# wongzbb/DiffMa-Diffusion-Mamba

Hardware: AMD Instinct MI355X
Metric: diffusion-steps/sec (DiffMa-L/2, 224x224, training; samples*steps/s) (higher is better)
Workload: dtype bf16 autocast (fp32 master weights, fp32 scan state); 1 GPU; DiffMa-L/2 DDP training step, 4x28x28 latents (196 tokens), batch 512/GPU; global_batch=512, seq_len=196, parallelism=dp1, gemm_tuning=file, world_size_seen_by_rccl=1

## Files before the change

diffma-diffusion-mamba_amd/csrc/scan_bwd.hip:

```cpp
#include "dm_common.h"
namespace dm {
int scan_bwd_f32(const dm_scan_bwd_args& a, const dm_scan_bwd_args* second, hipStream_t st);
int scan_bwd_bf16(const dm_scan_bwd_args& a, const dm_scan_bwd_args* second, hipStream_t st);
int scan_bwd_f16(const dm_scan_bwd_args& a, const dm_scan_bwd_args* second, hipStream_t st);
bool scan_bwd_takes_two(const dm_scan_bwd_args& a);

static int check_scan_bwd(const dm_scan_bwd_args& a) {
    if (!a.u || !a.delta || !a.dout || !a.A || !a.B || !a.C || !a.du || !a.ddelta || !a.dBC_partial || !a.dA_partial) {
        set_error("dm_selective_scan_bwd: null tensor pointer"); return DM_ERR_ARG;
    }
    if ((a.z != nullptr) != (a.dz != nullptr)) { set_error("dm_selective_scan_bwd: dz must be given iff z is"); return DM_ERR_ARG; }
    if (a.nseq <= 0 || a.dim <= 0 || a.seqlen <= 0 || a.ngroups <= 0) { set_error("dm_selective_scan_bwd: non-positive size"); return DM_ERR_ARG; }
    if (a.nseq > 65535) { set_error("dm_selective_scan_bwd: nseq %d > 65535", a.nseq); return DM_ERR_ARG; }
    if (a.ckpt_every != DM_SCAN_CKPT_EVERY) { set_error("dm_selective_scan_bwd: ckpt_every must be %d", DM_SCAN_CKPT_EVERY); return DM_ERR_ARG; }
    if (!a.ckpt) { set_error("dm_selective_scan_bwd: ckpt (the checkpoints written by dm_selective_scan_fwd) is required"); return DM_ERR_ARG; }
    if (a.ckpt && a.ckpt_dtype != (a.io_dtype == DM_BF16 ? DM_BF16 : DM_F32)) {
        set_error("dm_selective_scan_bwd: ckpt_dtype must be DM_BF16 for bf16 I/O and DM_F32 otherwise"); return DM_ERR_DTYPE;
    }
    if (a.u_sd != 1 || a.dt_sd != 1 || a.do_sd != 1 || a.du_sd != 1 || a.ddt_sd != 1 || (a.z && (a.z_sd != 1 || a.dz_sd != 1)) ||
        a.B_sn != 1 || a.C_sn != 1) {
        set_error("dm_selective_scan_bwd: needs token-major tensors (channel stride 1, state stride 1)"); return DM_ERR_LAYOUT;
    }
    if (a.dim % a.ngroups != 0 || (a.ngroups > 1 && (a.dim / a.ngroups) % WAVE != 0)) {
        set_error("dm_selective_scan_bwd: dim/ngroups must be a multiple of 64"); return DM_ERR_LAYOUT;
    }
    if (a.batch_per_dir > 0 && a.nseq % a.batch_per_dir != 0) { set_error("dm_selective_scan_bwd: nseq %% batch_per_dir != 0"); return DM_ERR_ARG; }
    if ((a.flags & DM_FLAG_DELTA_ACTIVATED) && (a.z || !a.z_row_index || a.dstate != 16 || (a.flags & (DM_FLAG_A_SHARED | DM_FLAG_DELTA_SOFTPLUS)))) {
        set_error("dm_selective_scan_bwd: DM_FLAG_DELTA_ACTIVATED is built for the mixer's call pattern (no z, row indices, d_state 16, no A_SHARED / DELTA_SOFTPLUS)");
        return DM_ERR_ARG;
    }
    if ((a.z_row_index == nullptr) != (a.out_row_index == nullptr)) {
        set_error("dm_selective_scan_bwd: z_row_index and out_row_index must both be set or both be NULL"); return DM_ERR_ARG;
    }
    return DM_OK;
}
static bool pairs_scan_bwd(const dm_scan_bwd_args& x, const dm_scan_bwd_args& y) {
    using A = dm_scan_bwd_args;
    return scan_bwd_takes_two(x) && mix_congruent(x, y, &A::u, &A::delta, &A::z, &A::dout, &A::B, &A::C, &A::A, &A::D, &A::delta_bias,
                                                  &A::z_row_index, &A::out_row_index, &A::ckpt, &A::du, &A::ddelta, &A::dz,
                                                  &A::dBC_partial, &A::dA_partial, &A::dD_partial, &A::dbias_partial);
}
static int run_scan_bwd(const dm_scan_bwd_args& a, const dm_scan_bwd_args* second, hipStream_t st) {
    switch (a.io_dtype) {
        case DM_F32: return scan_bwd_f32(a, second, st);
        case DM_BF16: return scan_bwd_bf16(a, second, st);
        case DM_F16: return scan_bwd_f16(a, second, st);
        default: set_error("dm_selective_scan_bwd: bad io_dtype %d", a.io_dtype); return DM_ERR_DTYPE;
    }
}
}

extern "C" int dm_selective_scan_bwd(const dm_scan_bwd_args* args, void* stream) {
    using namespace dm;
    if (!args) { set_error("dm_selective_scan_bwd: null args"); return DM_ERR_ARG; }
    const int rc = check_scan_bwd(*args);
    return rc ? rc : run_scan_bwd(*args, nullptr, (hipStream_t)stream);
}

extern "C" int dm_selective_scan_bwd_n(const dm_scan_bwd_args* args, int n, void* stream) {
    return dm::mix_run_n("dm_selective_scan_bwd_n", args, n, stream, dm::check_scan_bwd, dm::pairs_scan_bwd, dm::run_scan_bwd);
}
```

diffma-diffusion-mamba_amd/csrc/scan_bwd_impl.h:

```cpp
#pragma once
#include <type_traits>
#include "scan_bwd_step.h"

namespace dm {

constexpr int BWD_CK = 8;
constexpr int BWD_WAVES = 4;

__device__ __forceinline__ void swap32(float& a, float& b) {
    auto r = __builtin_amdgcn_permlane32_swap(__float_as_uint(a), __float_as_uint(b), false, false);
    a = __uint_as_float(r[0]);
    b = __uint_as_float(r[1]);
}
__device__ __forceinline__ void swap16(float& a, float& b) {
    auto r = __builtin_amdgcn_permlane16_swap(__float_as_uint(a), __float_as_uint(b), false, false);
    a = __uint_as_float(r[0]);
    b = __uint_as_float(r[1]);
}
template <int M>
__device__ __forceinline__ void lane_group_reduce(float (&v)[M]) {
    static_assert(M % 4 == 0, "need at least 2 states per lane");
#pragma unroll
    for (int i = 0; i < M / 2; ++i) { swap32(v[2 * i], v[2 * i + 1]); v[i] = v[2 * i] + v[2 * i + 1]; }
#pragma unroll
    for (int i = 0; i < M / 4; ++i) { swap16(v[2 * i], v[2 * i + 1]); v[i] = v[2 * i] + v[2 * i + 1]; }
}

typedef __attribute__((address_space(3))) const float* lds_cfptr;
typedef __attribute__((address_space(3))) const f32x4* lds_cf4ptr;
__device__ __forceinline__ lds_cfptr lds_opaque(lds_cfptr chunk_base) {
    asm volatile("" : "+v"(chunk_base));
    return chunk_base;
}
template <int NS>
__device__ __forceinline__ void lds_ld_vec(float (&v)[NS], lds_cfptr row) {
    if constexpr (NS % 4 == 0) {
#pragma unroll
        for (int k = 0; k < NS / 4; ++k) {
            const f32x4 t = ((lds_cf4ptr)row)[k];
            v[4 * k] = t.x; v[4 * k + 1] = t.y; v[4 * k + 2] = t.z; v[4 * k + 3] = t.w;
        }
    } else {
#pragma unroll
        for (int k = 0; k < NS; ++k) v[k] = row[k];
    }
}

template <typename T, typename TBC, int N, int SPLIT, bool HAS_Z, bool IDX, int DMODE, bool ASH = false>
__global__ __launch_bounds__(64 * BWD_WAVES) __attribute__((amdgpu_waves_per_eu(N <= 16 ? 2 : 1))) void scan_bwd_kernel(const dm_scan_bwd_args p) {
    constexpr int NS = N / SPLIT, NPL = NS / 2, CW = WAVE / SPLIT, CK = BWD_CK, SUB = DM_SCAN_CKPT_EVERY, M = 2 * NS, R = M / 4;
    constexpr int ES = (int)sizeof(T);
    constexpr bool MFMA_RED = std::is_same<T, bf16_t>::value && M % 16 == 0 && SPLIT <= 2;
    constexpr bool HALVES = MFMA_RED && SPLIT == 1 && N == 16;
    constexpr int NH = HALVES ? 2 : 1, NPH = NPL / NH;
    constexpr bool CACHE_A = HALVES && !ASH;
    constexpr bool LDS_AHEAD = HALVES && !HAS_Z;
    static_assert(N % SPLIT == 0 && NS % 2 == 0, "d_state/SPLIT must be even");
    static_assert(CK % SUB == 0, "chunk must be a whole number of sub-chunks");
    static_assert(R % 4 == 0, "lane-group totals are stored 4 registers at a time");
    constexpr int RED_HALF = WAVE * 4 + 4 * 8;
    constexpr int RED_ROW = (R / 4) * RED_HALF;
    __shared__ __attribute__((aligned(16))) float red_lds[BWD_WAVES][CK][RED_ROW];
    __shared__ __attribute__((aligned(16))) float bc_lds[2][CK][2 * N];

    const int tid = threadIdx.x;
    const int wave = tid >> 6, lane = tid & 63;
    const int c = lane / SPLIT, q = lane % SPLIT;
    const int d_raw = (blockIdx.x * BWD_WAVES + wave) * CW + c;
    const bool active = d_raw < p.dim;
    const int d = active ? d_raw : p.dim - 1;
    const int s = blockIdx.y;
    const int L = p.seqlen;
    const int bpd = (p.batch_per_dir > 0) ? p.batch_per_dir : p.nseq;
    const int dir = s / bpd;
    const int sb = s - dir * bpd;
    const int grp = (blockIdx.x * BWD_WAVES * CW) / (p.dim / p.ngroups);
    const int nwg = gridDim.x;
    const int nchunk = (L + CK - 1) / CK;

    const rsrc_t r_u = make_rsrc((const T*)p.u + (int64_t)s * p.u_ss);
    const rsrc_t r_dt = make_rsrc((const T*)p.delta + (int64_t)s * p.dt_ss);
    const rsrc_t r_z = make_rsrc(HAS_Z ? (const T*)p.z + (int64_t)sb * p.z_ss : nullptr);
    const rsrc_t r_g = make_rsrc((const T*)p.dout + (int64_t)((IDX && !(p.flags & DM_FLAG_DOUT_PER_SEQ)) ? sb : s) * p.do_ss);
    const rsrc_t r_du = make_rsrc_2g((T*)p.du + (int64_t)s * p.du_ss);
    const rsrc_t r_ddt = make_rsrc_2g((T*)p.ddelta + (int64_t)s * p.ddt_ss);
    const rsrc_t r_dz = make_rsrc_2g(HAS_Z ? (T*)p.dz + (int64_t)s * p.dz_ss : nullptr);
    const TBC* __restrict__ Bg = (const TBC*)p.B + (int64_t)s * p.B_ss + (int64_t)grp * p.B_sg;
    const TBC* __restrict__ Cg = (const TBC*)p.C + (int64_t)s * p.C_ss + (int64_t)grp * p.C_sg;
    constexpr bool CK_PACKED = std::is_same<T, bf16_t>::value;
    constexpr int CK_ROWS = CK_PACKED ? N / 2 : N;
    const int nck = (L + SUB - 1) / SUB;
    const rsrc_t r_ck = make_rsrc_2g(p.ckpt ? (const uint32_t*)p.ckpt + (int64_t)s * nck * CK_ROWS * p.dim : nullptr);
    const rsrc_t r_dbc = make_rsrc_2g(p.dBC_partial + (int64_t)s * L * gridDim.x * (2 * N));
    const int vo = d * ES;
    const int vo_st = (active && q == 0) ? vo : BIO_OOB;
    const int vo_ck = CK_PACKED ? (d * 4 + q * (CK_ROWS / SPLIT / 4) * p.dim * 4) * 4 : (d + q * (CK_ROWS / SPLIT) * p.dim) * 4;
    const int sl_u = (int)p.u_sl * ES, sl_dt = (int)p.dt_sl * ES, sl_z = (int)p.z_sl * ES, sl_g = (int)p.do_sl * ES;
    const int sl_du = (int)p.du_sl * ES, sl_ddt = (int)p.ddt_sl * ES, sl_dz = (int)p.dz_sl * ES;
    const int i_B_sl = (int)p.B_sl, i_C_sl = (int)p.C_sl;
    const cptr<int32_t> zidx = IDX ? as_const(p.z_row_index + (int64_t)dir * L) : nullptr;
    const cptr<int32_t> oidx = IDX ? as_const(p.out_row_index + (int64_t)dir * L) : nullptr;

    f32x2 A2[NPL];
#pragma unroll
    for (int k = 0; k < NPL; ++k) {
        A2[k].x = p.A[(int64_t)d * N + q * NS + 2 * k] * LOG2E;
        A2[k].y = p.A[(int64_t)d * N + q * NS + 2 * k + 1] * LOG2E;
    }
    const float Dv = p.D ? p.D[d] : 0.0f;
    const float bias = p.delta_bias ? p.delta_bias[d] : 0.0f;

    f32x2 carry[NPL], dA[NPL];
#pragma unroll
    for (int k = 0; k < NPL; ++k) { carry[k] = (f32x2){0.f, 0.f}; dA[k] = (f32x2){0.f, 0.f}; }
    float dD_acc = 0.f, dbias_acc = 0.f;

    u32x4_t sel_lo, sel_hi;
    if (MFMA_RED) mfma_selectors(lane, sel_lo, sel_hi);
    const int red_slot = lane * 4 + (lane >> 4) * 8;

    constexpr int BC_PER_THREAD = (CK * 2 * N + 64 * BWD_WAVES - 1) / (64 * BWD_WAVES);
    auto fetch_bc = [&](int chunk, uint32_t(&v)[BC_PER_THREAD]) {
#pragma unroll
        for (int i = 0; i < BC_PER_THREAD; ++i) {
            int e = tid + i * 64 * BWD_WAVES;
            e = (e < CK * 2 * N) ? e : CK * 2 * N - 1;
            const int j = e / (2 * N), cc = e % (2 * N);
            int l = chunk * CK + j;
            l = (l < L) ? l : L - 1;
            const TBC* src = (cc < N) ? Bg + l * i_B_sl + cc : Cg + l * i_C_sl + (cc - N);
            v[i] = io<TBC>::ld_raw(src);
        }
    };
    auto stash_bc = [&](int b, const uint32_t(&v)[BC_PER_THREAD]) {
#pragma unroll
        for (int i = 0; i < BC_PER_THREAD; ++i) {
            const int e = tid + i * 64 * BWD_WAVES;
            if (e < CK * 2 * N) bc_lds[b][e / (2 * N)][e % (2 * N)] = io<TBC>::cv(v[i]);
        }
    };
    auto flush_dbc = [&](int chunk) {
        const int l0 = chunk * CK;
        if constexpr (HALVES) {
            static_assert(CK * 2 * N == 64 * BWD_WAVES, "one output per thread");
            const int tq = tid & 3, g4 = (tid >> 2) & 7, j = tid >> 5;
            const float* base = &red_lds[0][j][(g4 >> 2) * RED_HALF + (16 * (g4 & 3) + 4 * tq) * 4 + (g4 & 3) * 8];
            f32x4 acc4 = {0.f, 0.f, 0.f, 0.f};
#pragma unroll
            for (int w = 0; w < BWD_WAVES; ++w)
#pragma unroll
                for (int t = 0; t < 4; ++t) acc4 += *reinterpret_cast<const f32x4*>(base + w * (CK * RED_ROW) + t * 4);
#pragma unroll
            for (int i = 0; i < 4; ++i) {
                float v = acc4[i];
                v += dpp<DPP_QUAD_SWAP>(v);
                v += dpp<DPP_QUAD_HALF>(v);
                acc4[i] = v;
            }
            const float mine = tq == 0 ? acc4[0] : (tq == 1 ? acc4[1] : (tq == 2 ? acc4[2] : acc4[3]));
            const int V = 4 * g4 + tq;
            const int col = (V & 8) ? N + 8 * (V >> 4) + (V & 7) : 8 * (V >> 4) + (V & 7);
            const int vo_p = (l0 + j < L) ? (((l0 + j) * nwg + (int)blockIdx.x) * (2 * N) + col) * 4 : BIO_OOB;
            __builtin_amdgcn_raw_buffer_store_b32(__float_as_uint(mine), r_dbc, vo_p, 0, 0);
            return;
        }
#pragma unroll
        for (int it = 0; it < BC_PER_THREAD; ++it) {
            const int e_ = tid + it * 64 * BWD_WAVES;
            const bool in = e_ < CK * 2 * N;
            const int e = in ? e_ : 0;
            const int j = e / (2 * N), cc = e % (2 * N);
            const int vo_p = (in && l0 + j < L) ? (((l0 + j) * nwg + (int)blockIdx.x) * (2 * N) + cc) * 4 : BIO_OOB;
            float acc = 0.f;
            const int n = (cc < N) ? cc : cc - N;
            const int qq = n / NS;
            const int vidx = (cc < N) ? n % NS : NS + n % NS;
            const int lane0 = (MFMA_RED ? 16 * ((vidx & 15) >> 2) : 32 * (vidx & 1) + 16 * ((vidx >> 1) & 1)) + qq;
            const int reg = MFMA_RED ? 4 * (vidx >> 4) + (vidx & 3) : (vidx >> 2);
#pragma unroll
            for (int w = 0; w < BWD_WAVES; ++w)
#pragma unroll
                for (int t = 0; t < 16 / SPLIT; ++t) acc += red_lds[w][j][(reg >> 2) * RED_HALF + (lane0 + SPLIT * t) * 4 + (lane0 >> 4) * 8 + (reg & 3)];
            __builtin_amdgcn_raw_buffer_store_b32(__float_as_uint(acc), r_dbc, vo_p, 0, 0);
        }
    };
    {
        uint32_t v[BC_PER_THREAD];
        fetch_bc(nchunk - 1, v);
        stash_bc(0, v);
    }
    __syncthreads();

    constexpr int H0W = CK_PACKED ? NPL : 2 * NPL;
    auto load_state = [&](int ci, uint32_t(&w)[H0W]) {
        const int slot_ = ckpt_slot(ci, L);
        const int vo_ = (slot_ < 0 || !p.ckpt) ? BIO_OOB : vo_ck;
        const int slot = slot_ < 0 ? 0 : slot_;
        if constexpr (CK_PACKED) {
            bio_ld_words<H0W>(w, r_ck, vo_, slot * p.dim * (N / 2) * 4, p.dim * 16);
        } else {
#pragma unroll
            for (int k = 0; k < NPL; ++k) {
                w[2 * k] = __builtin_amdgcn_raw_buffer_load_b32(r_ck, vo_, ((slot * N + 2 * k) * p.dim) * 4, 0);
                w[2 * k + 1] = __builtin_amdgcn_raw_buffer_load_b32(r_ck, vo_, ((slot * N + 2 * k + 1) * p.dim) * 4, 0);
            }
        }
    };
    auto unpack_state = [&](f32x2(&h)[NPH], const uint32_t(&w)[H0W], int hf) {
        unpack_ckpt<CK_PACKED>(h, w, hf * NPH);
    };
    static_assert(SUB == 4, "row-table entries of a sub-chunk travel in one 4-entry SGPR vector");
    constexpr int NSC = CK / SUB;
    typedef int i32x4_t __attribute__((ext_vector_type(4)));
    auto load_rows = [&](cptr<int32_t> tab, int ci) -> i32x4_t {
        const int lb = ci < 0 ? 0 : ci * SUB;
        i32x4_t r = {0, 0, 0, 0};
#pragma unroll
        for (int i = 0; i < SUB; ++i) {
            const int l = (lb + i < L) ? lb + i : L - 1;
            r[i] = IDX ? tab[(uint32_t)l] : l;
        }
        return r;
    };
    typename bio<T>::raw_t ru[SUB], rd[SUB], rg[SUB], rz[HAS_Z ? SUB : 1];
    uint32_t ck_nx[H0W];
    i32x4_t orow_is = load_rows(oidx, nchunk * NSC - 1), zrow_is = {0, 0, 0, 0};
    if (HAS_Z) zrow_is = load_rows(zidx, nchunk * NSC - 1);
    auto issue_sub = [&](int ci) {
        const int lb = ci < 0 ? 0 : ci * SUB;
#pragma unroll
        for (int i = 0; i < SUB; ++i) {
            const int l = (lb + i < L) ? lb + i : L - 1;
            ru[i] = bio<T>::ld_raw(r_u, vo, l * sl_u);
            rd[i] = bio<T>::ld_raw(r_dt, vo, l * sl_dt);
            if (HAS_Z) rz[i] = bio<T>::ld_raw(r_z, vo, zrow_is[i] * sl_z);
            rg[i] = bio<T>::ld_raw(r_g, vo, orow_is[i] * sl_g);
        }
        load_state(ci, ck_nx);
        orow_is = load_rows(oidx, ci - 1);
        if (HAS_Z) zrow_is = load_rows(zidx, ci - 1);
    };
    uint32_t ck_end[H0W];
    load_state(nchunk * NSC, ck_end);
    f32x2 hend[HALVES ? NH : 1][NPH];
    if constexpr (HALVES) {
#pragma unroll
        for (int hf = 0; hf < NH; ++hf) unpack_state(hend[hf], ck_end, hf);
    }
    i32x4_t zrow_nx = zrow_is;
    issue_sub(nchunk * NSC - 1);

    int buf = 0;
    for (int ch = nchunk - 1; ch >= 0; --ch) {
        const int l0 = ch * CK;
        const lds_cfptr bc_chunk = (lds_cfptr)(&bc_lds[0][0][0]) + (buf * CK * 2 * N + q * NS);
        uint32_t bc_next[BC_PER_THREAD];
        fetch_bc(ch > 0 ? ch - 1 : 0, bc_next);
#pragma unroll
        for (int sc = NSC - 1; sc >= 0; --sc) {
            const int ci = ch * NSC + sc;
            float uu[SUB], dl[SUB], zz[SUB], gg[SUB];
            uint32_t ck_cur[H0W];
            const i32x4_t zrow = zrow_nx;
#pragma unroll
            for (int i = 0; i < SUB; ++i) {
                const bool valid = (l0 + sc * SUB + i) < L;
                uu[i] = bio<T>::cv(ru[i]);
                dl[i] = activate_delta<DMODE>(bio<T>::cv(rd[i]), bias);
                zz[i] = HAS_Z ? bio<T>::cv(rz[i]) : 0.f;
                gg[i] = (valid && active) ? bio<T>::cv(rg[i]) : 0.f;
            }
#pragma unroll
            for (int k = 0; k < H0W; ++k) ck_cur[k] = ck_nx[k];
            zrow_nx = zrow_is;
            issue_sub(ci - 1);
            f32x2 GB2s[SUB], dlA2s[SUB], yp2s[HAS_Z ? SUB : 1];
#pragma unroll
            for (int hf = 0; hf < NH; ++hf) {
            const lds_cfptr bc_rec = lds_opaque(bc_chunk);
            auto fwd_step = [&](f32x2(&h)[NPH], int i, f32x2(&keep)[NPH]) {
                float Bv[2 * NPH];
                const lds_cfptr brow = bc_rec + ((sc * SUB + i) * 2 * N + hf * 2 * NPH);
                lds_ld_vec<2 * NPH>(Bv, brow);
                const float dlo = CACHE_A ? dl[i] : opaque(dl[i]);
                const float du = dlo * uu[i];
                const float a_sh = decay_shared<ASH>(A2[0], dlo);
#pragma unroll
                for (int k = 0; k < NPH; ++k) {
                    const f32x2 a = decay_pair<ASH>(A2[hf * NPH + k], dlo, a_sh);
                    if (CACHE_A) keep[k] = a;
                    recompute_pair(h[k], a, (f32x2){Bv[2 * k], Bv[2 * k + 1]}, du);
                }
            };
            f32x2 h[NPH];
            unpack_state(h, ck_cur, hf);
            f32x2 hs[SUB][NPH];
            f32x2 aa[CACHE_A ? SUB - 1 : 1][NPH];
#pragma unroll
            for (int i = 0; i < SUB; ++i) {
#pragma unroll
                for (int k = 0; k < NPH; ++k) hs[i][k] = h[k];
                if (i < SUB - 1) fwd_step(h, i, aa[CACHE_A ? i : 0]);
            }
            if constexpr (HALVES) {
#pragma unroll
                for (int k = 0; k < NPH; ++k) { h[k] = hend[hf][k]; hend[hf][k] = hs[0][k]; }
            } else {
                unpack_state(h, ck_end, hf);
            }
            const lds_cfptr bc_swp = lds_opaque(bc_chunk);
            float Bn[2 * NPH], Cn[2 * NPH];
            if constexpr (LDS_AHEAD) {
// ... 34 lines not shown
#pragma unroll
                for (int k = 0; k < NPH; ++k) {
                    const int kk = hf * NPH + k;
                    const f32x2 bb = {Bv[2 * k], Bv[2 * k + 1]}, cc = {Cv[2 * k], Cv[2 * k + 1]};
                    const f32x2 a = (CACHE_A && i < SUB - 1) ? aa[CACHE_A ? i : 0][k] : decay_pair<ASH>(A2[kk], dlo, a_rev);
                    f32x2 dBp, dCp;
                    adjoint_pair<HAS_Z, true>(h[k], hs[i][k], carry[kk], dA[kk], yp2, GB2, dlA2, A2[kk], a, bb, cc, gy, du, dlo, dBp, dCp);
                    if constexpr (MFMA_RED) {
                        pk_all[k] = pack_bf16(dBp);
                        pk_all[NPH + k] = pack_bf16(dCp);
                    } else {
                        red[2 * k] = dBp.x;
                        red[2 * k + 1] = dBp.y;
                        red[NS + 2 * k] = dCp.x;
                        red[NS + 2 * k + 1] = dCp.y;
                    }
                }
                if (hf < NH - 1) { GB2s[i] = GB2; dlA2s[i] = dlA2; if (HAS_Z) yp2s[i] = yp2; }
                if (hf == NH - 1) {
                float ddl, duv, ypre, dDi;
                step_outputs<DMODE, SPLIT>(yp2, GB2, dlA2, uu[i], dlo, gy, Dv, ddl, duv, ypre, dDi);
                if (q == 0) {
                    dD_acc += dDi;
                    dbias_acc += ddl;
                }
                const int vo_s = valid ? vo_st : BIO_OOB;
                bio<T>::st_cv(r_du, vo_s, l * sl_du, duv);
                bio<T>::st_cv(r_ddt, vo_s, l * sl_ddt, ddl);
                if (HAS_Z) {
                    const float dzv = gate_grad(g, ypre, zz[i], sz);
                    bio<T>::st_cv(r_dz, vo_s, zrow[i] * sl_dz, dzv);
                }
                }
                if constexpr (MFMA_RED) {
#pragma unroll
                    for (int g16 = 0; g16 < M / 16 / NH; ++g16)
                        *reinterpret_cast<f32x4*>(&red_lds[wave][j][(NH == 2 ? hf : g16) * RED_HALF + red_slot]) = group_sum16(sel_lo, sel_hi, pk_all + 8 * g16);
                } else {
                    lane_group_reduce<M>(red);
#pragma unroll
                    for (int r4 = 0; r4 < R / 4; ++r4)
                        *reinterpret_cast<f32x4*>(&red_lds[wave][j][r4 * RED_HALF + red_slot]) = (f32x4){red[4 * r4], red[4 * r4 + 1], red[4 * r4 + 2], red[4 * r4 + 3]};
                }
            }
            }
#pragma unroll
            for (int k = 0; k < H0W; ++k) ck_end[k] = ck_cur[k];
        }
        __syncthreads();
        flush_dbc(ch);
        if (ch > 0) stash_bc(buf ^ 1, bc_next);
        __syncthreads();
        buf ^= 1;
    }
    if (active) {
        const int64_t pss_a = p.part_ss ? p.part_ss : (int64_t)p.dim * N, pss_d = p.part_ss ? p.part_ss : (int64_t)p.dim;
        float* dAp = p.dA_partial + (int64_t)s * pss_a + (int64_t)d * N + q * NS;
#pragma unroll
        for (int k = 0; k < NPL; ++k) {
            dAp[2 * k] = dA[k].x;
            dAp[2 * k + 1] = dA[k].y;
        }
        if (q == 0) {
            if (p.dD_partial) p.dD_partial[(int64_t)s * pss_d + d] = dD_acc;
            if (p.dbias_partial) p.dbias_partial[(int64_t)s * pss_d + d] = dbias_acc;
        }
    }
}

template <int N> struct bwd_split { static constexpr int value = N >= 32 ? (N >= 64 ? N / 16 : 2) : 1; };

template <int N, bool HAS_Z, bool IDX, typename F>
static void with_bwd_variant(int flags, F f) {
    const bool sp = (flags & DM_FLAG_DELTA_SOFTPLUS) != 0;
    if constexpr ((N == 16 || N == 64 || N == 128) && HAS_Z && IDX) {
        if ((flags & DM_FLAG_A_SHARED) && sp) return f(std::integral_constant<int, 1>{}, std::true_type{});
    }
    if constexpr (N == 16 && !HAS_Z && IDX) {
        if (flags & DM_FLAG_DELTA_ACTIVATED) return f(std::integral_constant<int, 2>{}, std::false_type{});
    }
    if (sp) f(std::integral_constant<int, 1>{}, std::false_type{});
    else f(std::integral_constant<int, 0>{}, std::false_type{});
}

template <typename T, typename TBC, int N>
static int launch_bwd(const dm_scan_bwd_args& a, hipStream_t st) {
    constexpr int SPLIT = bwd_split<N>::value, WGCH = (WAVE / SPLIT) * BWD_WAVES;
    dim3 grid((a.dim + WGCH - 1) / WGCH, a.nseq);
    with_z_idx(a, [&](auto hz, auto ix) {
        with_bwd_variant<N, hz.value, ix.value>(a.flags, [&](auto dmode, auto ash) {
            hipLaunchKernelGGL((scan_bwd_kernel<T, TBC, N, SPLIT, hz.value, ix.value, dmode.value, ash.value>), grid, dim3(WAVE * BWD_WAVES), 0, st, a);
        });
    });
    return launch_status("dm_selective_scan_bwd");
}

template <typename T, typename TBC>
static int bwd_dispatch_n(const dm_scan_bwd_args& a, hipStream_t st) {
    switch (a.dstate) {
        case 16: return launch_bwd<T, TBC, 16>(a, st);
#ifndef DM_FAST_BUILD
        case 8: return launch_bwd<T, TBC, 8>(a, st);
        case 32: return launch_bwd<T, TBC, 32>(a, st);
        case 64: return launch_bwd<T, TBC, 64>(a, st);
        case 128: return launch_bwd<T, TBC, 128>(a, st);
#endif
        default: set_error("dm_selective_scan_bwd: d_state=%d not instantiated (8,16,32,64,128)", a.dstate); return DM_ERR_DSTATE;
    }
}

template <typename T>
static int bwd_dispatch_bc(const dm_scan_bwd_args& a, hipStream_t st) {
    if (a.bc_dtype == DM_F32) return bwd_dispatch_n<T, float>(a, st);
    if (a.bc_dtype == a.io_dtype) return bwd_dispatch_n<T, T>(a, st);
    set_error("dm_selective_scan_bwd: bc_dtype %d must be fp32 or equal io_dtype %d", a.bc_dtype, a.io_dtype);
    return DM_ERR_DTYPE;
}

}
```

diffma-diffusion-mamba_amd/hip_ops.py:

```python
from __future__ import annotations

import ctypes
import os
import threading

import torch

from . import _lib
from ._lib import (DM_BF16, DM_F16, DM_F32, DM_FLAG_A_SHARED, DM_FLAG_DELTA_ACTIVATED, DM_FLAG_DX_MERGED, DM_FLAG_PARTIAL_COMPACT, DM_FLAG_OUT_ACCUMULATE, DM_FLAG_DELTA_SOFTPLUS, DM_FLAG_DOUT_PER_SEQ, DM_FLAG_SCAN_CHUNKED, DM_FLAG_SCAN_SEQUENTIAL, DM_FLAG_SILU, dm_blend_args, dm_gate_head_args, dm_dtproj_bwd_args, dm_conv_bwd_args, dm_rmsnorm_merge_args, dm_colsum_args, dm_sum_partials_args,
                   dm_conv_fwd_args, dm_conv_xproj_bwd_args, dm_conv_xproj_fwd_args, dm_diffusion_step_args, dm_ln_mod_args, dm_ssd_bwd_args, dm_ssd_fwd_args, dm_merge_args, dm_gate_bwd_args, dm_dtproj_args, dm_scan_bwd_args, dm_scan_fwd_args, dm_gemm_args, dm_repack_args, dm_training_loss_args)

_DT = {torch.float32: DM_F32, torch.bfloat16: DM_BF16, torch.float16: DM_F16}
SCAN_CKPT_EVERY = _lib.DM_SCAN_CKPT_EVERY


def union_length(intervals):
    total, cur_s, cur_e = 0.0, None, None
    for s0, e0 in sorted(intervals):
        if cur_e is None or s0 > cur_e:
            if cur_e is not None:
                total += cur_e - cur_s
            cur_s, cur_e = s0, e0
        else:
            cur_e = max(cur_e, e0)
# ... 210 lines not shown
    return a


def scan_fwd(u, delta, A, Bm, Cm, D=None, z=None, delta_bias=None, delta_softplus=True, *,
             z_row_index=None, out_row_index=None, batch_per_dir=0, out=None, ckpt=None,
             ckpt_every=SCAN_CKPT_EVERY, last_state=None, ngroups=1, a_shared=False, variant=None, acc_dirs=False,
             delta_activated=False):
    _require_gpu(u, delta, A, Bm, Cm, z)
    S, L, Dm = u.shape
    N = A.shape[1]
    if acc_dirs:
        Bd = batch_per_dir
        ndir = S // Bd
        if out is None:
            out = torch.empty((Bd, L, Dm), dtype=u.dtype, device=u.device)
        for k in range(ndir):
            sl = slice(k * Bd, (k + 1) * Bd)
            _scan_fwd_launch(u[sl], delta[sl], A, Bm[sl], Cm[sl], D, z, delta_bias, delta_softplus, z_row_index[k:k + 1],
                             out_row_index[k:k + 1], 0, out, None if ckpt is None else ckpt[sl], ckpt_every, None, ngroups, False,
                             "sequential", k > 0)
        return out
    if out is None:
        out = torch.empty((S, L, Dm), dtype=u.dtype, device=u.device)
    return _scan_fwd_launch(u, delta, A, Bm, Cm, D, z, delta_bias, delta_softplus, z_row_index, out_row_index, batch_per_dir, out, ckpt,
                            ckpt_every, last_state, ngroups, a_shared, variant, False, delta_activated)


def _scan_fwd_launch(u, delta, A, Bm, Cm, D, z, delta_bias, delta_softplus, z_row_index, out_row_index, batch_per_dir, out, ckpt,
                     ckpt_every, last_state, ngroups, a_shared, variant, accumulate, delta_activated=False):
    S, L, Dm = u.shape
    N = A.shape[1]
    A, D, delta_bias = _f32c(A), _f32c(D), _f32c(delta_bias)
    a = _scan_args(dm_scan_fwd_args(), u, delta, A, Bm, Cm, D, z, delta_bias, delta_softplus, delta_activated, z_row_index, out_row_index,
                   batch_per_dir, ckpt, ckpt_every, ngroups, a_shared, variant, DM_FLAG_OUT_ACCUMULATE if accumulate else 0)
    a.out, a.last_state = _ptr(out), _ptr(last_state)
    a.o_ss, a.o_sl, a.o_sd = out.stride()
    nbytes = scan_fwd_algorithmic_bytes(S, Dm, L, N, u.element_size(), Bm.element_size(), z is not None)
    design = nbytes
    if accumulate:
        design += S * Dm * L * u.element_size()
    if ckpt is not None:
        design += scan_nchunk(L, ckpt_every) * S * ckpt.shape[2] * ckpt.shape[3] * 4
    _launch("dm_selective_scan_fwd", a, u, nbytes, design)
    return out


def scan_bwd_partial_shape(S, L, Dm, N, flags=0):
    gc = _lib.load().dm_scan_bwd_launch_group_channels(S, Dm, L, N, flags)
    if gc <= 0:
        raise _lib.DiffmaHipError(f"selective-scan backward is not built for d_state={N}")
    return (S, L, (Dm + gc - 1) // gc, 2 * N)


def scan_bwd(u, delta, A, Bm, Cm, D, z, delta_bias, dout, ckpt, delta_softplus=True, *,
             z_row_index=None, out_row_index=None, batch_per_dir=0, ckpt_every=SCAN_CKPT_EVERY,
             ngroups=1, dz_out=None, dout_per_seq=False, du_out=None, a_shared=False, dbc_out=None, variant=None,
             delta_activated=False):
    _require_gpu(u, delta, A, Bm, Cm, z, dout, ckpt)
    S, L, Dm = u.shape
    N = A.shape[1]
    A32, D32, b32 = _f32c(A), _f32c(D), _f32c(delta_bias)
    a = _scan_args(dm_scan_bwd_args(), u, delta, A32, Bm, Cm, D32, z, b32, delta_softplus, delta_activated, z_row_index, out_row_index,
                   batch_per_dir, ckpt, ckpt_every, ngroups, a_shared, variant, DM_FLAG_DOUT_PER_SEQ if dout_per_seq else 0)
    dbc_shape = scan_bwd_partial_shape(S, L, Dm, N, a.flags)
    nw = dbc_shape[2]
    dev = u.device
    du = du_out if du_out is not None else torch.empty_like(u)
    ddelta = torch.empty((S, L, Dm), dtype=u.dtype, device=dev)
    dz = None
    if z is not None:
        dz = dz_out if dz_out is not None else torch.empty((S, L, Dm), dtype=u.dtype, device=dev)
    dBC = torch.empty(dbc_shape, dtype=torch.float32, device=dev)
    want_dD, want_db = D is not None, (delta_bias is not None or delta_activated)
    pcols = Dm * N + Dm * (int(want_dD) + int(want_db))
    part = torch.empty((S, pcols), dtype=torch.float32, device=dev)
    dA = part[:, :Dm * N]
    dD = part[:, Dm * N:Dm * N + Dm] if want_dD else None
    dbias = part[:, pcols - Dm:] if want_db else None
    a.part_ss = pcols
    a.dout = _ptr(dout)
    a.du, a.ddelta, a.dz = _ptr(du), _ptr(ddelta), _ptr(dz)
    a.dBC_partial, a.dA_partial = _ptr(dBC), _ptr(dA)
    a.dD_partial, a.dbias_partial = _ptr(dD), _ptr(dbias)
    if z is not None:
        a.dz_ss, a.dz_sl, a.dz_sd = dz.stride()
    a.do_ss, a.do_sl, a.do_sd = dout.stride()
    a.du_ss, a.du_sl, a.du_sd = du.stride()
    a.ddt_ss, a.ddt_sl, a.ddt_sd = ddelta.stride()
    nbytes = scan_bwd_algorithmic_bytes(S, Dm, L, N, u.element_size(), z is not None)
    design = nbytes + 2 * S * N * L * Bm.element_size() + S * L * (nw - 1) * 2 * N * 4 + 4 * S * Dm * (N + 2) \
        + (scan_nchunk(L, ckpt_every) - 1 + (L % ckpt_every == 0)) * S * ckpt.shape[2] * ckpt.shape[3] * 4
    _launch("dm_selective_scan_bwd", a, u, nbytes, design)
    if dbc_out is not None:
        dBCs = sum_partials(dBC.view(S * L, nw, 2 * N), dbc_out)
    else:
        dBCs = sum_partials(dBC.view(S * L, nw, 2 * N), torch.empty((S, L, 2 * N), dtype=torch.float32, device=dev))
    dB, dC = dBCs[..., :N], dBCs[..., N:]
    psum = colsum(part)
    return (du, ddelta, dz, dB, dC, psum[:Dm * N].view(Dm, N), psum[Dm * N:Dm * N + Dm] if want_dD else None,
            psum[pcols - Dm:] if want_db else None)


def sum_partials(parts, out):
    M, nw, C = parts.shape
    o2 = out.reshape(M, C) if out.is_contiguous() else None
    if o2 is None:
        st = out.stride()
        sr = st[-2]
        ok = out.stride(-1) == 1 and all(st[i] == st[i + 1] * out.shape[i + 1] for i in range(out.dim() - 2))
        o2 = out.as_strided((M, C), (sr, 1)) if ok else None
    es = out.element_size()
    if (o2 is None or C % 4 or not parts.is_contiguous() or parts.dtype != torch.float32 or out.dtype not in _DT
            or o2.data_ptr() % (4 * es) or o2.stride(0) % 4):
        _pair_flush()
        out.copy_(parts.sum(dim=1).view(out.shape))
        return out
    a = dm_sum_partials_args()
    a.rows, a.nw, a.cols = M, nw, C
    a.out_dtype = _DT[out.dtype]
    setattr(a, "in", _ptr(parts))
    a.out = _ptr(o2)
    a.out_sr = o2.stride(0)
    _launch("dm_sum_partials", a, parts, M * C * (nw * 4 + es))
    return out


COLSUM_SPLIT = os.environ.get("DIFFMA_COLSUM_SPLIT", "1") == "1"


def colsum(x):
    R, C = x.shape
    if C % 4 != 0 or not x.is_contiguous() or x.dtype != torch.float32:
        _pair_flush()
        return x.sum(0)
    wgs = (C // 4 + 63) // 64
    if COLSUM_SPLIT and R >= 256 and wgs < 48:
        rb = 1
        while rb < 32 and R % (2 * rb) == 0 and wgs * rb < 192 and R // (2 * rb) >= 16:
            rb *= 2
        if rb > 1:
            return _colsum_launch(_colsum_launch(x.view(R // rb, rb * C)).view(rb, C))
    return _colsum_launch(x)

# ... 792 lines not shown
```

include/diffma_hip.h:

```cpp
#ifndef DIFFMA_HIP_H
#define DIFFMA_HIP_H

#include <stdint.h>

#ifdef __cplusplus
extern "C" {
#endif

#define DM_ABI_VERSION 33

typedef enum {
    DM_OK = 0,
    DM_ERR_ARG = -1,
    DM_ERR_LAYOUT = -2,
    DM_ERR_DTYPE = -3,
    DM_ERR_DSTATE = -4,
    DM_ERR_LAUNCH = -5
} dm_status;

typedef enum { DM_F32 = 0, DM_BF16 = 1, DM_F16 = 2 } dm_dtype;

enum {
    DM_FLAG_DELTA_SOFTPLUS = 1,
    DM_FLAG_SILU = 2,
    DM_FLAG_A_SHARED = 8,
    DM_FLAG_DOUT_PER_SEQ = 4,
    DM_FLAG_SCAN_SEQUENTIAL = 16,
    DM_FLAG_SCAN_CHUNKED = 32,
    DM_FLAG_OUT_ACCUMULATE = 64,
    DM_FLAG_DX_MERGED = 256,
    DM_FLAG_PARTIAL_COMPACT = 512,
    DM_FLAG_DELTA_ACTIVATED = 128
};

typedef struct {
    int32_t batch, channels, hw, T;
    int32_t out_dtype, _pad;
    int32_t row_sqrt_ac, row_sqrt_1mac, row_post_logvar, row_log_betas, row_sqrt_recip_ac, row_sqrt_recipm1_ac, row_coef1, row_coef2;
    const void *model_out;
    const float *x_start, *x_t, *noise;
    const int64_t *t;
    const float *tables;
    float *x_t_out;
    float *mse, *vb, *loss, *grad;
    const float *g_eps, *g_v;
    void *grad_out;
} dm_training_loss_args;

int dm_q_sample(const dm_training_loss_args *args, void *stream);
int dm_training_loss(const dm_training_loss_args *args, void *stream);
int dm_training_loss_bwd(const dm_training_loss_args *args, void *stream);

typedef struct {
    float *p, *m, *v;
    const float *g;
    float *ema;
    float *step;
    int64_t n;
} dm_adamw_tensor;

typedef struct {
    const dm_adamw_tensor *tensors;
// ... 19 lines not shown
    int32_t flags;
    int32_t ckpt_every;
    int32_t ckpt_dtype;
    const void *u, *delta, *z;
    void *out;
    const void *B, *C;
    const float *A;
    const float *D;
    const float *delta_bias;
    const int32_t *z_row_index;
    const int32_t *out_row_index;
    void *ckpt;
    float *last_state;
    int64_t u_ss, u_sl, u_sd;
    int64_t dt_ss, dt_sl, dt_sd;
    int64_t z_ss, z_sl, z_sd;
    int64_t o_ss, o_sl, o_sd;
    int64_t B_ss, B_sl, B_sg, B_sn;
    int64_t C_ss, C_sl, C_sg, C_sn;
} dm_scan_fwd_args;

int dm_selective_scan_fwd(const dm_scan_fwd_args *args, void *stream);

typedef struct {
    int32_t nseq, dim, seqlen, dstate;
    int32_t ngroups;
    int32_t batch_per_dir;
    int32_t io_dtype;
    int32_t bc_dtype;
    int32_t flags;
    int32_t ckpt_every;
    int32_t ckpt_dtype;
    const void *u, *delta, *z, *dout;
    const void *B, *C;
    const float *A, *D, *delta_bias;
    const int32_t *z_row_index;
    const int32_t *out_row_index;
    const void *ckpt;
    void *du, *ddelta, *dz;
    float *dBC_partial;
    float *dA_partial;
    float *dD_partial;
    float *dbias_partial;
    int64_t u_ss, u_sl, u_sd;
    int64_t dt_ss, dt_sl, dt_sd;
    int64_t z_ss, z_sl, z_sd;
    int64_t do_ss, do_sl, do_sd;
    int64_t B_ss, B_sl, B_sg, B_sn;
    int64_t C_ss, C_sl, C_sg, C_sn;
    int64_t du_ss, du_sl, du_sd;
    int64_t ddt_ss, ddt_sl, ddt_sd;
    int64_t dz_ss, dz_sl, dz_sd;
    int64_t part_ss;
} dm_scan_bwd_args;

int dm_selective_scan_bwd(const dm_scan_bwd_args *args, void *stream);
int dm_scan_bwd_group_channels(int dstate);
int dm_scan_bwd_launch_group_channels(int nseq, int dim, int seqlen, int dstate, int flags);

typedef struct {
    int32_t batch, dim, seqlen, width, ndir;
    int32_t io_dtype, w_dtype;
    int32_t flags;
    const void *x;
    const void *weight;
    const void *bias;
    const int32_t *row_index;
    void *out;
    int64_t x_sb, x_sl, x_sd;
    int64_t o_ss, o_sl, o_sd;
} dm_conv_fwd_args;

int dm_gather_conv1d_fwd(const dm_conv_fwd_args *args, void *stream);

typedef struct {
    int32_t batch, dim, seqlen, width, ndir;
    int32_t io_dtype, w_dtype;
    int32_t flags;
    int32_t nchunk;
    const void *x, *weight, *bias, *dout;
    const int32_t *row_index;
    void *dx;
    float *dw_partial, *db_partial;
    int64_t x_sb, x_sl, x_sd;
    int64_t do_ss, do_sl, do_sd;
    int64_t dx_ss, dx_sl, dx_sd;
    int64_t part_ss;
} dm_conv_bwd_args;

int dm_gather_conv1d_bwd(const dm_conv_bwd_args *args, void *stream);
int dm_conv_nchunk(int seqlen);

typedef struct {
    int32_t batch, dim, seqlen, width, ndir;
    int32_t io_dtype, w_dtype;
    int32_t flags;
    int32_t nproj;
    int32_t _pad;
    const void *x;
    const void *weight;
    const void *bias;
    const int32_t *row_index;
    const void *wx;
    void *out;
    void *xdbl;
    int64_t x_sb, x_sl, x_sd;
// ... 297 lines not shown
```

Baseline: 2543 samples*steps/s.

## Let scan backward workgroups process multiple sequences and peel partial last chunk

Adds a seq_per_wg parameter so each scan-backward workgroup can loop over several sequences, re-deriving its per-sequence buffer descriptors from the kernel-argument segment, and shrinks the dA/dD/dbias partials buffer to match. The aim is to cut workgroup launch and partial-sum reduction overhead when the grid is much larger than the resident slots. It also peels a final half-filled chunk so that only its one live sub-chunk is processed. With the default SEQ_PER_WG of 1 the grid is unchanged, so mainly the peeling and the added per-sequence setup and register pressure affect default runs.

```diff
diff --git a/diffma-diffusion-mamba_amd/csrc/scan_bwd.hip b/diffma-diffusion-mamba_amd/csrc/scan_bwd.hip
--- a/diffma-diffusion-mamba_amd/csrc/scan_bwd.hip
+++ b/diffma-diffusion-mamba_amd/csrc/scan_bwd.hip
@@ -11,6 +11,7 @@
     }
     if ((a.z != nullptr) != (a.dz != nullptr)) { set_error("dm_selective_scan_bwd: dz must be given iff z is"); return DM_ERR_ARG; }
     if (a.nseq <= 0 || a.dim <= 0 || a.seqlen <= 0 || a.ngroups <= 0) { set_error("dm_selective_scan_bwd: non-positive size"); return DM_ERR_ARG; }
+    if (a.seq_per_wg < 0) { set_error("dm_selective_scan_bwd: seq_per_wg %d < 0", a.seq_per_wg); return DM_ERR_ARG; }
     if (a.nseq > 65535) { set_error("dm_selective_scan_bwd: nseq %d > 65535", a.nseq); return DM_ERR_ARG; }
     if (a.ckpt_every != DM_SCAN_CKPT_EVERY) { set_error("dm_selective_scan_bwd: ckpt_every must be %d", DM_SCAN_CKPT_EVERY); return DM_ERR_ARG; }
     if (!a.ckpt) { set_error("dm_selective_scan_bwd: ckpt (the checkpoints written by dm_selective_scan_fwd) is required"); return DM_ERR_ARG; }
diff --git a/diffma-diffusion-mamba_amd/csrc/scan_bwd_impl.h b/diffma-diffusion-mamba_amd/csrc/scan_bwd_impl.h
--- a/diffma-diffusion-mamba_amd/csrc/scan_bwd_impl.h
+++ b/diffma-diffusion-mamba_amd/csrc/scan_bwd_impl.h
@@ -6,6 +6,9 @@
 
 constexpr int BWD_CK = 8;
 constexpr int BWD_WAVES = 4;
+#ifndef DM_SCAN_BWD_PEEL
+#define DM_SCAN_BWD_PEEL 1
+#endif
 
 __device__ __forceinline__ void swap32(float& a, float& b) {
     auto r = __builtin_amdgcn_permlane32_swap(__float_as_uint(a), __float_as_uint(b), false, false);
@@ -44,6 +47,21 @@
 #pragma unroll
         for (int k = 0; k < NS; ++k) v[k] = row[k];
     }
+}
+
+typedef const __attribute__((address_space(4))) dm_scan_bwd_args* kargs_t;
+__device__ __forceinline__ int opaque_int(int x) {
+    asm volatile("" : "+v"(x));
+    return x;
+}
+__device__ __forceinline__ int opaque_uniform(int x) {
+    asm volatile("" : "+s"(x));
+    return x;
+}
+__device__ __forceinline__ kargs_t seq_args() {
+    kargs_t a = (kargs_t)__builtin_amdgcn_kernarg_segment_ptr();
+    asm volatile("" : "+s"(a));
+    return a;
 }
 
 template <typename T, typename TBC, int N, int SPLIT, bool HAS_Z, bool IDX, int DMODE, bool ASH = false>
@@ -69,37 +87,47 @@
     const int d_raw = (blockIdx.x * BWD_WAVES + wave) * CW + c;
     const bool active = d_raw < p.dim;
     const int d = active ? d_raw : p.dim - 1;
-    const int s = blockIdx.y;
+    const int spw = p.seq_per_wg > 1 ? p.seq_per_wg : 1;
+    const int s_first = blockIdx.y * spw;
+    const int s_last = (s_first + spw < p.nseq ? s_first + spw : p.nseq) - 1;
     const int L = p.seqlen;
     const int bpd = (p.batch_per_dir > 0) ? p.batch_per_dir : p.nseq;
-    const int dir = s / bpd;
-    const int sb = s - dir * bpd;
     const int grp = (blockIdx.x * BWD_WAVES * CW) / (p.dim / p.ngroups);
     const int nwg = gridDim.x;
     const int nchunk = (L + CK - 1) / CK;
-
-    const rsrc_t r_u = make_rsrc((const T*)p.u + (int64_t)s * p.u_ss);
-    const rsrc_t r_dt = make_rsrc((const T*)p.delta + (int64_t)s * p.dt_ss);
-    const rsrc_t r_z = make_rsrc(HAS_Z ? (const T*)p.z + (int64_t)sb * p.z_ss : nullptr);
-    const rsrc_t r_g = make_rsrc((const T*)p.dout + (int64_t)((IDX && !(p.flags & DM_FLAG_DOUT_PER_SEQ)) ? sb : s) * p.do_ss);
-    const rsrc_t r_du = make_rsrc_2g((T*)p.du + (int64_t)s * p.du_ss);
-    const rsrc_t r_ddt = make_rsrc_2g((T*)p.ddelta + (int64_t)s * p.ddt_ss);
-    const rsrc_t r_dz = make_rsrc_2g(HAS_Z ? (T*)p.dz + (int64_t)s * p.dz_ss : nullptr);
-    const TBC* __restrict__ Bg = (const TBC*)p.B + (int64_t)s * p.B_ss + (int64_t)grp * p.B_sg;
-    const TBC* __restrict__ Cg = (const TBC*)p.C + (int64_t)s * p.C_ss + (int64_t)grp * p.C_sg;
+    constexpr int NSC = CK / SUB;
     constexpr bool CK_PACKED = std::is_same<T, bf16_t>::value;
     constexpr int CK_ROWS = CK_PACKED ? N / 2 : N;
     const int nck = (L + SUB - 1) / SUB;
-    const rsrc_t r_ck = make_rsrc_2g(p.ckpt ? (const uint32_t*)p.ckpt + (int64_t)s * nck * CK_ROWS * p.dim : nullptr);
-    const rsrc_t r_dbc = make_rsrc_2g(p.dBC_partial + (int64_t)s * L * gridDim.x * (2 * N));
+    const int nsub = DM_SCAN_BWD_PEEL ? nck : nchunk * NSC;
+
+    rsrc_t r_u, r_dt, r_z, r_g, r_ck, r_du, r_ddt, r_dz, r_dbc;
+    cptr<int32_t> zidx = nullptr, oidx = nullptr;
+    const TBC* __restrict__ Bg;
+    const TBC* __restrict__ Cg;
+    auto seek = [&](int s) {
+        const kargs_t a = seq_args();
+        const int dir = s / bpd, sb = s - dir * bpd;
+        r_u = make_rsrc((const T*)a->u + (int64_t)s * a->u_ss);
+        r_dt = make_rsrc((const T*)a->delta + (int64_t)s * a->dt_ss);
+        r_z = make_rsrc(HAS_Z ? (const T*)a->z + (int64_t)sb * a->z_ss : nullptr);
+        r_g = make_rsrc((const T*)a->dout + (int64_t)((IDX && !(a->flags & DM_FLAG_DOUT_PER_SEQ)) ? sb : s) * a->do_ss);
+        r_ck = make_rsrc_2g(a->ckpt ? (const uint32_t*)a->ckpt + (int64_t)s * nck * CK_ROWS * a->dim : nullptr);
+        r_du = make_rsrc_2g((T*)a->du + (int64_t)s * a->du_ss);
+        r_ddt = make_rsrc_2g((T*)a->ddelta + (int64_t)s * a->ddt_ss);
+        r_dz = make_rsrc_2g(HAS_Z ? (T*)a->dz + (int64_t)s * a->dz_ss : nullptr);
+        r_dbc = make_rsrc_2g(a->dBC_partial + (int64_t)s * L * nwg * (2 * N));
+        zidx = (IDX && HAS_Z) ? as_const(a->z_row_index + (int64_t)dir * L) : nullptr;
+        oidx = IDX ? as_const(a->out_row_index + (int64_t)dir * L) : nullptr;
+        Bg = (const TBC*)a->B + (int64_t)s * a->B_ss + (int64_t)grp * a->B_sg;
+        Cg = (const TBC*)a->C + (int64_t)s * a->C_ss + (int64_t)grp * a->C_sg;
+    };
     const int vo = d * ES;
     const int vo_st = (active && q == 0) ? vo : BIO_OOB;
     const int vo_ck = CK_PACKED ? (d * 4 + q * (CK_ROWS / SPLIT / 4) * p.dim * 4) * 4 : (d + q * (CK_ROWS / SPLIT) * p.dim) * 4;
     const int sl_u = (int)p.u_sl * ES, sl_dt = (int)p.dt_sl * ES, sl_z = (int)p.z_sl * ES, sl_g = (int)p.do_sl * ES;
     const int sl_du = (int)p.du_sl * ES, sl_ddt = (int)p.ddt_sl * ES, sl_dz = (int)p.dz_sl * ES;
     const int i_B_sl = (int)p.B_sl, i_C_sl = (int)p.C_sl;
-    const cptr<int32_t> zidx = IDX ? as_const(p.z_row_index + (int64_t)dir * L) : nullptr;
-    const cptr<int32_t> oidx = IDX ? as_const(p.out_row_index + (int64_t)dir * L) : nullptr;
 
     f32x2 A2[NPL];
 #pragma unroll
@@ -123,7 +151,7 @@
     auto fetch_bc = [&](int chunk, uint32_t(&v)[BC_PER_THREAD]) {
 #pragma unroll
         for (int i = 0; i < BC_PER_THREAD; ++i) {
-            int e = tid + i * 64 * BWD_WAVES;
+            int e = opaque_int(tid) + i * 64 * BWD_WAVES;
             e = (e < CK * 2 * N) ? e : CK * 2 * N - 1;
             const int j = e / (2 * N), cc = e % (2 * N);
             int l = chunk * CK + j;
@@ -184,13 +212,6 @@
             __builtin_amdgcn_raw_buffer_store_b32(__float_as_uint(acc), r_dbc, vo_p, 0, 0);
         }
     };
-    {
-        uint32_t v[BC_PER_THREAD];
-        fetch_bc(nchunk - 1, v);
-        stash_bc(0, v);
-    }
-    __syncthreads();
-
     constexpr int H0W = CK_PACKED ? NPL : 2 * NPL;
     auto load_state = [&](int ci, uint32_t(&w)[H0W]) {
         const int slot_ = ckpt_slot(ci, L);
@@ -210,7 +231,6 @@
         unpack_ckpt<CK_PACKED>(h, w, hf * NPH);
     };
     static_assert(SUB == 4, "row-table entries of a sub-chunk travel in one 4-entry SGPR vector");
-    constexpr int NSC = CK / SUB;
     typedef int i32x4_t __attribute__((ext_vector_type(4)));
     auto load_rows = [&](cptr<int32_t> tab, int ci) -> i32x4_t {
         const int lb = ci < 0 ? 0 : ci * SUB;
@@ -224,8 +244,7 @@
     };
     typename bio<T>::raw_t ru[SUB], rd[SUB], rg[SUB], rz[HAS_Z ? SUB : 1];
     uint32_t ck_nx[H0W];
-    i32x4_t orow_is = load_rows(oidx, nchunk * NSC - 1), zrow_is = {0, 0, 0, 0};
-    if (HAS_Z) zrow_is = load_rows(zidx, nchunk * NSC - 1);
+    i32x4_t orow_is, zrow_is = {0, 0, 0, 0};
     auto issue_sub = [&](int ci) {
         const int lb = ci < 0 ? 0 : ci * SUB;
 #pragma unroll
@@ -241,23 +260,18 @@
         if (HAS_Z) zrow_is = load_rows(zidx, ci - 1);
     };
     uint32_t ck_end[H0W];
-    load_state(nchunk * NSC, ck_end);
     f32x2 hend[HALVES ? NH : 1][NPH];
-    if constexpr (HALVES) {
-#pragma unroll
-        for (int hf = 0; hf < NH; ++hf) unpack_state(hend[hf], ck_end, hf);
-    }
-    i32x4_t zrow_nx = zrow_is;
-    issue_sub(nchunk * NSC - 1);
+    i32x4_t zrow_nx;
 
     int buf = 0;
-    for (int ch = nchunk - 1; ch >= 0; --ch) {
+    auto run_chunk = [&](const int ch, auto nlive) {
+        constexpr int NLIVE = decltype(nlive)::value;
         const int l0 = ch * CK;
         const lds_cfptr bc_chunk = (lds_cfptr)(&bc_lds[0][0][0]) + (buf * CK * 2 * N + q * NS);
         uint32_t bc_next[BC_PER_THREAD];
         fetch_bc(ch > 0 ? ch - 1 : 0, bc_next);
 #pragma unroll
-        for (int sc = NSC - 1; sc >= 0; --sc) {
+        for (int sc = NLIVE - 1; sc >= 0; --sc) {
             const int ci = ch * NSC + sc;
             float uu[SUB], dl[SUB], zz[SUB], gg[SUB];
             uint32_t ck_cur[H0W];
@@ -398,9 +412,39 @@
         if (ch > 0) stash_bc(buf ^ 1, bc_next);
         __syncthreads();
         buf ^= 1;
+    };
+    for (int s = s_first; s <= s_last; ++s) {
+        seek(s);
+        {
+            uint32_t v[BC_PER_THREAD];
+            fetch_bc(opaque_uniform(nchunk) - 1, v);
+            stash_bc(buf, v);
+        }
+        orow_is = load_rows(oidx, nsub - 1);
+        if (HAS_Z) zrow_is = load_rows(zidx, nsub - 1);
+        load_state(nsub, ck_end);
+        zrow_nx = zrow_is;
+        issue_sub(nsub - 1);
+#pragma unroll
+        for (int k = 0; k < NPL; ++k) carry[k] = (f32x2){0.f, 0.f};
+        if constexpr (HALVES) {
+#pragma unroll
+            for (int hf = 0; hf < NH; ++hf) unpack_state(hend[hf], ck_end, hf);
+        }
+        __syncthreads();
+        int ch = opaque_uniform(nchunk) - 1;
+        if (nsub - ch * NSC < NSC) {
+            static_assert(NSC == 2, "a chunk that is not whole has one live sub-chunk");
+            run_chunk(ch, std::integral_constant<int, 1>{});
+            --ch;
+        }
+        for (; ch >= 0; --ch) run_chunk(ch, std::integral_constant<int, NSC>{});
     }
     if (active) {
         const int64_t pss_a = p.part_ss ? p.part_ss : (int64_t)p.dim * N, pss_d = p.part_ss ? p.part_ss : (int64_t)p.dim;
+        const int s = blockIdx.y;
+        const int tid = opaque_int(threadIdx.x);
+        const int d = (blockIdx.x * BWD_WAVES + (tid >> 6)) * CW + (tid & 63) / SPLIT;
         float* dAp = p.dA_partial + (int64_t)s * pss_a + (int64_t)d * N + q * NS;
 #pragma unroll
         for (int k = 0; k < NPL; ++k) {
@@ -432,7 +476,8 @@
 template <typename T, typename TBC, int N>
 static int launch_bwd(const dm_scan_bwd_args& a, hipStream_t st) {
     constexpr int SPLIT = bwd_split<N>::value, WGCH = (WAVE / SPLIT) * BWD_WAVES;
-    dim3 grid((a.dim + WGCH - 1) / WGCH, a.nseq);
+    const int spw = a.seq_per_wg > 1 ? a.seq_per_wg : 1;
+    dim3 grid((a.dim + WGCH - 1) / WGCH, (a.nseq + spw - 1) / spw);
     with_z_idx(a, [&](auto hz, auto ix) {
         with_bwd_variant<N, hz.value, ix.value>(a.flags, [&](auto dmode, auto ash) {
             hipLaunchKernelGGL((scan_bwd_kernel<T, TBC, N, SPLIT, hz.value, ix.value, dmode.value, ash.value>), grid, dim3(WAVE * BWD_WAVES), 0, st, a);
diff --git a/diffma-diffusion-mamba_amd/hip_ops.py b/diffma-diffusion-mamba_amd/hip_ops.py
--- a/diffma-diffusion-mamba_amd/hip_ops.py
+++ b/diffma-diffusion-mamba_amd/hip_ops.py
@@ -286,10 +286,31 @@
     return (S, L, (Dm + gc - 1) // gc, 2 * N)
 
 
+SCAN_BWD_SLOTS = 512
+SCAN_BWD_SEQ_PER_WG = 1
+SCAN_BWD_SEQ_PER_WG_ENV = "DIFFMA_SCAN_BWD_SEQ_PER_WG"
+
+
+def scan_bwd_seq_per_wg(nseq, nwg_per_seq, sequential=True):
+    if not sequential:
+        return 1
+    env = os.environ.get(SCAN_BWD_SEQ_PER_WG_ENV, "")
+    if env:
+        return min(max(1, int(env)), nseq)
+    wgs = nseq * nwg_per_seq
+    if wgs < 2 * SCAN_BWD_SLOTS:
+        return 1
+    return max(1, min(SCAN_BWD_SEQ_PER_WG, nseq, wgs // SCAN_BWD_SLOTS))
+
+
+def scan_bwd_part_shape(nseq, seq_per_wg, Dm, N, want_dD=True, want_dbias=True):
+    return ((nseq + seq_per_wg - 1) // seq_per_wg, Dm * N + Dm * (int(want_dD) + int(want_dbias)))
+
+
 def scan_bwd(u, delta, A, Bm, Cm, D, z, delta_bias, dout, ckpt, delta_softplus=True, *,
              z_row_index=None, out_row_index=None, batch_per_dir=0, ckpt_every=SCAN_CKPT_EVERY,
              ngroups=1, dz_out=None, dout_per_seq=False, du_out=None, a_shared=False, dbc_out=None, variant=None,
-             delta_activated=False):
+             delta_activated=False, ddelta_out=None):
     _require_gpu(u, delta, A, Bm, Cm, z, dout, ckpt)
     S, L, Dm = u.shape
     N = A.shape[1]
@@ -300,14 +321,16 @@
     nw = dbc_shape[2]
     dev = u.device
     du = du_out if du_out is not None else torch.empty_like(u)
-    ddelta = torch.empty((S, L, Dm), dtype=u.dtype, device=dev)
+    ddelta = ddelta_out if ddelta_out is not None else torch.empty((S, L, Dm), dtype=u.dtype, device=dev)
     dz = None
     if z is not None:
         dz = dz_out if dz_out is not None else torch.empty((S, L, Dm), dtype=u.dtype, device=dev)
     dBC = torch.empty(dbc_shape, dtype=torch.float32, device=dev)
     want_dD, want_db = D is not None, (delta_bias is not None or delta_activated)
-    pcols = Dm * N + Dm * (int(want_dD) + int(want_db))
-    part = torch.empty((S, pcols), dtype=torch.float32, device=dev)
+    lib = _lib.load()
+    a.seq_per_wg = scan_bwd_seq_per_wg(S, nw, sequential=lib.dm_scan_bwd_launch_group_channels(S, Dm, L, N, a.flags) == lib.dm_scan_bwd_group_channels(N))
+    prows, pcols = scan_bwd_part_shape(S, a.seq_per_wg, Dm, N, want_dD, want_db)
+    part = torch.empty((prows, pcols), dtype=torch.float32, device=dev)
     dA = part[:, :Dm * N]
     dD = part[:, Dm * N:Dm * N + Dm] if want_dD else None
     dbias = part[:, pcols - Dm:] if want_db else None
@@ -322,7 +345,7 @@
     a.du_ss, a.du_sl, a.du_sd = du.stride()
     a.ddt_ss, a.ddt_sl, a.ddt_sd = ddelta.stride()
     nbytes = scan_bwd_algorithmic_bytes(S, Dm, L, N, u.element_size(), z is not None)
-    design = nbytes + 2 * S * N * L * Bm.element_size() + S * L * (nw - 1) * 2 * N * 4 + 4 * S * Dm * (N + 2) \
+    design = nbytes + 2 * S * N * L * Bm.element_size() + S * L * (nw - 1) * 2 * N * 4 + 4 * prows * Dm * (N + 2) \
         + (scan_nchunk(L, ckpt_every) - 1 + (L % ckpt_every == 0)) * S * ckpt.shape[2] * ckpt.shape[3] * 4
     _launch("dm_selective_scan_bwd", a, u, nbytes, design)
     if dbc_out is not None:
diff --git a/include/diffma_hip.h b/include/diffma_hip.h
--- a/include/diffma_hip.h
+++ b/include/diffma_hip.h
@@ -7,7 +7,7 @@
 extern "C" {
 #endif
 
-#define DM_ABI_VERSION 33
+#define DM_ABI_VERSION 34
 
 typedef enum {
     DM_OK = 0,
@@ -133,6 +133,8 @@
     int64_t ddt_ss, ddt_sl, ddt_sd;
     int64_t dz_ss, dz_sl, dz_sd;
     int64_t part_ss;
+    int32_t seq_per_wg;
+    int32_t _pad_seq;
 } dm_scan_bwd_args;
 
 int dm_selective_scan_bwd(const dm_scan_bwd_args *args, void *stream);
```

Result: no change. 2548 samples*steps/s, median of 2 (+0.2%).
